# fenghansen/YOND_public

Measured on AMD Instinct MI355X. Metric: Bayer megapixels/sec end-to-end (NLE+VST+denoise+iVST), higher is better.
Workload: dtype f32 (3x3 convolutions: f32 operands as two f16 halves -- 22-23 significant bits -- on the f16 MFMA, 3 products per f32 product, f32 accumulate; per-layer error vs float64 asserted <= 2x the f32 direct kernel's and <= 2e-5 of max|ref| (tests/test_hip_conv.py; measured 1.3e-6 vs 1.5e-6), whole frame v

## Files before the change

yond_public_amd/csrc/conv_misc.hip:

```cpp
#include "common.h"

template <int TH>
__global__ __launch_bounds__(256) void conv_in_kernel(const float* __restrict__ x, const float* __restrict__ ub,
                                                      int H, int W, int Cout, const float* __restrict__ wpk,
                                                      const float* __restrict__ bias, float slope,
                                                      float* __restrict__ dst, int out_p4) {
    constexpr int IH = TH + 2, IW = 34, MW = TH / 4;
    __shared__ __attribute__((aligned(16))) float s_in[IH * IW * 4];
    __shared__ __attribute__((aligned(16))) float s_w[5 * 2 * 32 * 4];
    const int tid = threadIdx.x, lane = tid & 63, wave = tid >> 6, li = lane & 31, lh = lane >> 5;
    const int nct = Cout / 32;
    const int ntx = (W + 31) / 32;
    int b = blockIdx.x;
    const int ct = b % nct;
    b /= nct;
    const int tx = b % ntx, ty = b / ntx;
    const int n = blockIdx.y;
    const int ox0 = tx * 32, oy0 = ty * TH;
    const float u = ub ? ub[n] : 1.0f;
    for (int it = tid; it < IH * IW; it += 256) {
        const int py = it / IW, px = it % IW;
        const int gy = oy0 - 1 + py, gx = ox0 - 1 + px;
        f32x4 v = {0.0f, 0.0f, 0.0f, 0.0f};
        if (gy >= 0 && gy < H && gx >= 0 && gx < W) {
            v = *(const f32x4*)(x + ((size_t)(n * H + gy) * W + gx) * 4);
            if (ub) { v[0] /= u; v[1] /= u; v[2] /= u; v[3] /= u; }
        }
        *(f32x4*)(s_in + it * 4) = v;
    }
    for (int it = tid; it < 5 * 2 * 32; it += 256)
        *(f32x4*)(s_w + it * 4) = *(const f32x4*)(wpk + (size_t)ct * 1280 + it * 4);
    __syncthreads();

    f32x16 acc[MW];
#pragma unroll
    for (int m = 0; m < MW; ++m)
#pragma unroll
        for (int r = 0; r < 16; ++r) acc[m][r] = 0.0f;
#pragma unroll
    for (int up = 0; up < 5; ++up) {
        int tap = 2 * up + lh;
        if (tap > 8) tap = 8;
        const int dy = tap / 3, dx = tap % 3;
        const f32x4 bb = *(const f32x4*)(s_w + ((up * 2 + lh) * 32 + li) * 4);
#pragma unroll
        for (int m = 0; m < MW; ++m) {
            const f32x4 a = *(const f32x4*)(s_in + ((wave * MW + m + dy) * IW + li + dx) * 4);
#pragma unroll
            for (int t = 0; t < 4; ++t) acc[m] = __builtin_amdgcn_mfma_f32_32x32x2f32(bb[t], a[t], acc[m], 0, 0, 0);
        }
    }
    const int ox = ox0 + li;
#pragma unroll
    for (int m = 0; m < MW; ++m) {
        const int oy = oy0 + wave * MW + m;
        if (oy < H && ox < W) {
            float* op = out_p4 ? dst + (((size_t)n * (Cout / 4) + ct * 8 + lh) * H * W + (size_t)oy * W + ox) * 4
                               : dst + ((size_t)(n * H + oy) * W + ox) * Cout + ct * 32 + 4 * lh;
            const size_t gstep = out_p4 ? (size_t)8 * H * W : 8;
#pragma unroll
            for (int g = 0; g < 4; ++g) {
                const f32x4 zero = {0.0f, 0.0f, 0.0f, 0.0f};
                const f32x4 bv = bias ? *(const f32x4*)(bias + ct * 32 + 4 * lh + 8 * g) : zero;
                f32x4 v;
#pragma unroll
                for (int e = 0; e < 4; ++e) {
                    const float x = acc[m][4 * g + e] + bv[e];
                    v[e] = x > 0.0f ? x : x * slope;
                }
                *(f32x4*)(op + g * gstep) = v;
            }
        }
    }
}

extern "C" int yond_pack_conv_in_weight_f32(const float* w, int cout, float* dst) {
    if (!w || !dst || cout % 32 != 0) return YOND_EINVAL;
    size_t o = 0;
    for (int ct = 0; ct < cout / 32; ++ct)
        for (int up = 0; up < 5; ++up)
            for (int h = 0; h < 2; ++h)
                for (int j = 0; j < 32; ++j)
                    for (int e = 0; e < 4; ++e) {
                        const int tap = 2 * up + h, co = ct * 32 + j;
                        dst[o++] = tap < 9 ? w[((size_t)co * 4 + e) * 9 + tap] : 0.0f;
                    }
    return YOND_OK;
}

extern "C" int yond_conv_in_f32(const float* x, const float* ub, int N, int H, int W, int Cout, const float* wpk,
                                const float* bias, float slope, float* dst, int out_fmt, void* stream) {
    if (!x || !wpk || !dst || N <= 0 || H <= 0 || W <= 0 || N > 65535) return YOND_EINVAL;
    if (out_fmt != YOND_FMT_NHWC_F32 && out_fmt != YOND_FMT_PLANES4) return YOND_EINVAL;
    if (Cout % 32 != 0) return YOND_EUNSUPPORTED;
    constexpr int TH = 8;
    dim3 grid((Cout / 32) * ((W + 31) / 32) * ((H + TH - 1) / TH), N);
    hipLaunchKernelGGL(conv_in_kernel<TH>, grid, dim3(256), 0, (hipStream_t)stream, x, ub, H, W, Cout, wpk, bias, slope, dst,
                       out_fmt == YOND_FMT_PLANES4 ? 1 : 0);
    YOND_LAUNCH_CHECK();
    return YOND_OK;
}

__global__ __launch_bounds__(256) void conv_out_kernel(const float* __restrict__ feat, int Cin,
                                                       const float* __restrict__ w, const float* __restrict__ bias,
                                                       const float* __restrict__ x, const float* __restrict__ ub,
                                                       size_t npix_per_image, float* __restrict__ dst) {
    const int n = blockIdx.y;
    const int part = threadIdx.x & 7;
    const float u = ub ? ub[n] : 1.0f;
    const size_t stride = (size_t)gridDim.x * 32;
    for (size_t p = (size_t)blockIdx.x * 32 + (threadIdx.x >> 3); p < npix_per_image; p += stride) {
        const size_t gp = (size_t)n * npix_per_image + p;
        const float* f = feat + gp * Cin + part * 4;
        float o0 = 0.f, o1 = 0.f, o2 = 0.f, o3 = 0.f;
        for (int c = 0; c < Cin; c += 32) {
            const f32x4 v = *(const f32x4*)(f + c);
            const int cb = c + part * 4;
#pragma unroll
            for (int e = 0; e < 4; ++e) {
                o0 = fmaf(v[e], w[0 * Cin + cb + e], o0);
                o1 = fmaf(v[e], w[1 * Cin + cb + e], o1);
                o2 = fmaf(v[e], w[2 * Cin + cb + e], o2);
                o3 = fmaf(v[e], w[3 * Cin + cb + e], o3);
            }
        }
#pragma unroll
        for (int m = 1; m < 8; m <<= 1) {
            o0 += __shfl_xor(o0, m); o1 += __shfl_xor(o1, m); o2 += __shfl_xor(o2, m); o3 += __shfl_xor(o3, m);
        }
        if (part == 0) {
            if (bias) { o0 += bias[0]; o1 += bias[1]; o2 += bias[2]; o3 += bias[3]; }
            if (x) {
                f32x4 xv = *(const f32x4*)(x + gp * 4);
                if (ub) { xv[0] /= u; xv[1] /= u; xv[2] /= u; xv[3] /= u; }
                o0 += xv[0]; o1 += xv[1]; o2 += xv[2]; o3 += xv[3];
            }
            if (ub) { o0 *= u; o1 *= u; o2 *= u; o3 *= u; }
            f32x4 o = {o0, o1, o2, o3};
            *(f32x4*)(dst + gp * 4) = o;
        }
    }
}

extern "C" int yond_conv_out_f32(const float* feat, int Cin, const float* w, const float* bias, const float* x,
                                 const float* ub, int N, int H, int W, float* dst, void* stream) {
    if (!feat || !w || !dst || N <= 0 || H <= 0 || W <= 0 || N > 65535) return YOND_EINVAL;
    if (Cin % 32 != 0) return YOND_EUNSUPPORTED;
    const size_t npix = (size_t)H * W;
    size_t nb = (npix + 31) / 32;
    if (nb > 256 * 32) nb = 256 * 32;
    dim3 grid((unsigned)nb, N);
    hipLaunchKernelGGL(conv_out_kernel, grid, dim3(256), 0, (hipStream_t)stream, feat, Cin, w, bias, x, ub, npix, dst);
    YOND_LAUNCH_CHECK();
    return YOND_OK;
}

__global__ __launch_bounds__(256) void maxpool2_kernel(const float* __restrict__ src, int H, int W, int C,
                                                       float* __restrict__ dst, size_t total4) {
    const size_t i = (size_t)blockIdx.x * 256 + threadIdx.x;
    if (i >= total4) return;
    const int c4 = C / 4;
    const int Ho = H / 2, Wo = W / 2;
    const int c = (int)(i % c4);
    size_t p = i / c4;
    const int ox = (int)(p % Wo);
    p /= Wo;
    const int oy = (int)(p % Ho);
    const int n = (int)(p / Ho);
    const float* s = src + (((size_t)(n * H + 2 * oy) * W + 2 * ox) * C) + c * 4;
    const f32x4 a = *(const f32x4*)s, b2 = *(const f32x4*)(s + C);
    const f32x4 c2 = *(const f32x4*)(s + (size_t)W * C), d2 = *(const f32x4*)(s + (size_t)W * C + C);
    f32x4 o;
#pragma unroll
    for (int e = 0; e < 4; ++e) o[e] = fmaxf(fmaxf(a[e], b2[e]), fmaxf(c2[e], d2[e]));
    *(f32x4*)(dst + i * 4) = o;
}

extern "C" int yond_maxpool2_f32(const float* src, int N, int H, int W, int C, float* dst, void* stream) {
    if (!src || !dst || N <= 0 || H < 2 || W < 2 || (H & 1) || (W & 1) || C % 4 != 0) return YOND_EINVAL;
    const size_t total4 = (size_t)N * (H / 2) * (W / 2) * (C / 4);
    hipLaunchKernelGGL(maxpool2_kernel, dim3((unsigned)((total4 + 255) / 256)), dim3(256), 0, (hipStream_t)stream, src, H, W, C, dst, total4);
    YOND_LAUNCH_CHECK();
    return YOND_OK;
}

template <int STAGE>
__global__ __launch_bounds__(256) void film_kernel(const YondFilmDesc* __restrict__ descs, const float* __restrict__ t,
                                                   const float* __restrict__ ub) {
    __shared__ float s_h[1024];
    const YondFilmDesc d = descs[blockIdx.y];
    const int n = blockIdx.z;
    const int C = d.C;
    if ((int)blockIdx.x * 32 >= C) return;
    const int tid = threadIdx.x, lane = tid & 63, wave = tid >> 6;
    float tv = t[n];
    if (ub) tv = tv / ub[n];
    const float* Wm;
    if (STAGE == 0) {
        for (int c = tid; c < C; c += 256) s_h[c] = silu_f(fmaf(d.w_a0[c], tv, d.b_a0[c]));
        Wm = d.w_a2;
    } else {
        if (d.kind == 0) {
            for (int c = tid; c < C; c += 256) s_h[c] = silu_f(d.s1[(size_t)n * d.ld + c]);
        } else {
            for (int c = tid; c < C; c += 256) s_h[c] = silu_f(fmaf(d.w_b0[c], tv, d.b_b0[c]));
        }
        Wm = d.w_b;
    }
    __syncthreads();
    for (int row0 = blockIdx.x * 32; row0 < C; row0 += gridDim.x * 32) {
    float acc8[8];
#pragma unroll
    for (int i = 0; i < 8; ++i) acc8[i] = 0.0f;
    const int rbase = row0 + wave * 8;
    for (int j = lane; j < C; j += 64) {
        const float hj = s_h[j];
#pragma unroll
        for (int i = 0; i < 8; ++i) {
            const int row = min(rbase + i, C - 1);
            acc8[i] = fmaf(Wm[(size_t)row * C + j], hj, acc8[i]);
        }
    }
#pragma unroll
    for (int i = 0; i < 8; ++i) {
        const int row = rbase + i;
        float s = acc8[i];
#pragma unroll
        for (int o = 32; o > 0; o >>= 1) s += __shfl_xor(s, o);
        if (row >= C) continue;
        if (lane == 0) {
            const size_t o = (size_t)n * d.ld + row;
            if (STAGE == 0) {
                d.s1[o] = s + d.b_a2[row];
            } else {
                const float m2 = s + d.b_b[row];
                const float m1 = d.s1[o];
                if (d.kind == 0) {
                    d.t1[o] = fmaf(d.cb1[row], m1, m2);
                    d.s2[o] = 1.0f;
                    d.t2[o] = d.cb2[row];
                } else {
                    d.t1[o] = d.cb1[row] * m1;
                    d.s2[o] = m2;
                    d.t2[o] = d.cb2[row] * m2;
                }
            }
        }
    }
    }
}

extern "C" int yond_film_f32(const YondFilmDesc* descs, int nblocks, const float* t, const float* ub, int N, void* stream) {
    if (!descs || !t || nblocks <= 0 || N <= 0 || N > 65535 || nblocks > 65535) return YOND_EINVAL;
    dim3 grid(N >= 8 ? (unsigned)yond_exp_long("YOND_FILM_GX", 8) : 1024 / 32, nblocks, N);
    hipLaunchKernelGGL(film_kernel<0>, grid, dim3(256), 0, (hipStream_t)stream, descs, t, ub);
    YOND_LAUNCH_CHECK();
    hipLaunchKernelGGL(film_kernel<1>, grid, dim3(256), 0, (hipStream_t)stream, descs, t, ub);
    YOND_LAUNCH_CHECK();
    return YOND_OK;
}
```

Before: 2612.

## Make conv_in persistent with double-buffered input tiles and prefetch

```diff
diff --git a/yond_public_amd/csrc/conv_misc.hip b/yond_public_amd/csrc/conv_misc.hip
--- a/yond_public_amd/csrc/conv_misc.hip
+++ b/yond_public_amd/csrc/conv_misc.hip
@@ -1,76 +1,112 @@
 #include "common.h"
 
 template <int TH>
-__global__ __launch_bounds__(256) void conv_in_kernel(const float* __restrict__ x, const float* __restrict__ ub,
-                                                      int H, int W, int Cout, const float* __restrict__ wpk,
+__global__ __launch_bounds__(256) __attribute__((amdgpu_waves_per_eu(5, 5))) void conv_in_kernel(const float* __restrict__ x, const float* __restrict__ ub,
+                                                      int N, int H, int W, int Cout, const float* __restrict__ wpk,
                                                       const float* __restrict__ bias, float slope,
                                                       float* __restrict__ dst, int out_p4) {
     constexpr int IH = TH + 2, IW = 34, MW = TH / 4;
-    __shared__ __attribute__((aligned(16))) float s_in[IH * IW * 4];
-    __shared__ __attribute__((aligned(16))) float s_w[5 * 2 * 32 * 4];
+    constexpr int NLD = (IH * IW + 255) / 256;
+    __shared__ __attribute__((aligned(16))) float s_in[2][IH * IW * 4];
     const int tid = threadIdx.x, lane = tid & 63, wave = tid >> 6, li = lane & 31, lh = lane >> 5;
-    const int nct = Cout / 32;
-    const int ntx = (W + 31) / 32;
-    int b = blockIdx.x;
-    const int ct = b % nct;
-    b /= nct;
-    const int tx = b % ntx, ty = b / ntx;
-    const int n = blockIdx.y;
-    const int ox0 = tx * 32, oy0 = ty * TH;
-    const float u = ub ? ub[n] : 1.0f;
-    for (int it = tid; it < IH * IW; it += 256) {
-        const int py = it / IW, px = it % IW;
-        const int gy = oy0 - 1 + py, gx = ox0 - 1 + px;
-        f32x4 v = {0.0f, 0.0f, 0.0f, 0.0f};
-        if (gy >= 0 && gy < H && gx >= 0 && gx < W) {
-            v = *(const f32x4*)(x + ((size_t)(n * H + gy) * W + gx) * 4);
-            if (ub) { v[0] /= u; v[1] /= u; v[2] /= u; v[3] /= u; }
-        }
-        *(f32x4*)(s_in + it * 4) = v;
-    }
+    const int ct = blockIdx.y;
+    const int ntx = (W + 31) / 32, nty = (H + TH - 1) / TH;
+    const int per_img = ntx * nty, total = N * per_img;
+    int t = blockIdx.x;
+    if (t >= total) return;
+    __shared__ __attribute__((aligned(16))) float s_w[5 * 2 * 32 * 4 + 32];
     for (int it = tid; it < 5 * 2 * 32; it += 256)
         *(f32x4*)(s_w + it * 4) = *(const f32x4*)(wpk + (size_t)ct * 1280 + it * 4);
+    if (tid < 32) s_w[1280 + tid] = bias ? bias[ct * 32 + tid] : 0.0f;
+    struct Tile { int n, ox0, oy0; };
+    auto tile_of = [&](int tt) {
+        Tile r;
+        r.n = tt / per_img;
+        const int q = tt - r.n * per_img, ty = q / ntx;
+        r.ox0 = (q - ty * ntx) * 32;
+        r.oy0 = ty * TH;
+        return r;
+    };
+    f32x4 v[NLD];
+    float u = 1.0f;
+    auto fetch = [&](const Tile& tl) {
+#pragma unroll
+        for (int k = 0; k < NLD; ++k) {
+            const int it = min(tid + k * 256, IH * IW - 1);
+            const int py = it / IW, px = it % IW;
+            const int gy = min(max(tl.oy0 - 1 + py, 0), H - 1), gx = min(max(tl.ox0 - 1 + px, 0), W - 1);
+            v[k] = *(const f32x4*)(x + ((size_t)(tl.n * H + gy) * W + gx) * 4);
+        }
+        if (ub) u = ub[tl.n];
+    };
+    auto stage = [&](const Tile& tl, float* s) {
+#pragma unroll
+        for (int k = 0; k < NLD; ++k) {
+            const int it = tid + k * 256;
+            if (it >= IH * IW) continue;
+            const int py = it / IW, px = it % IW;
+            const int gy = tl.oy0 - 1 + py, gx = tl.ox0 - 1 + px;
+            f32x4 a = {0.0f, 0.0f, 0.0f, 0.0f};
+            if (gy >= 0 && gy < H && gx >= 0 && gx < W) {
+                a = v[k];
+                if (ub) { a[0] /= u; a[1] /= u; a[2] /= u; a[3] /= u; }
+            }
+            *(f32x4*)(s + it * 4) = a;
+        }
+    };
+    Tile cur = tile_of(t);
+    fetch(cur);
+    stage(cur, s_in[0]);
     __syncthreads();
-
-    f32x16 acc[MW];
-#pragma unroll
-    for (int m = 0; m < MW; ++m)
-#pragma unroll
-        for (int r = 0; r < 16; ++r) acc[m][r] = 0.0f;
-#pragma unroll
-    for (int up = 0; up < 5; ++up) {
-        int tap = 2 * up + lh;
-        if (tap > 8) tap = 8;
-        const int dy = tap / 3, dx = tap % 3;
-        const f32x4 bb = *(const f32x4*)(s_w + ((up * 2 + lh) * 32 + li) * 4);
+    for (int buf = 0;; buf ^= 1) {
+        const int tn = t + gridDim.x;
+        const Tile nxt = tile_of(tn);
+        if (tn < total) fetch(nxt);
+        const float* si = s_in[buf];
+        f32x16 acc[MW];
+#pragma unroll
+        for (int m = 0; m < MW; ++m)
+#pragma unroll
+            for (int r = 0; r < 16; ++r) acc[m][r] = 0.0f;
+#pragma unroll
+        for (int up = 0; up < 5; ++up) {
+            int tap = 2 * up + lh;
+            if (tap > 8) tap = 8;
+            const int dy = tap / 3, dx = tap % 3;
+            const f32x4 bb = *(const f32x4*)(s_w + ((up * 2 + lh) * 32 + li) * 4);
+#pragma unroll
+            for (int m = 0; m < MW; ++m) {
+                const f32x4 a = *(const f32x4*)(si + ((wave * MW + m + dy) * IW + li + dx) * 4);
+#pragma unroll
+                for (int e = 0; e < 4; ++e) acc[m] = __builtin_amdgcn_mfma_f32_32x32x2f32(bb[e], a[e], acc[m], 0, 0, 0);
+            }
+        }
+        if (tn < total) stage(nxt, s_in[buf ^ 1]);
+        const int ox = cur.ox0 + li;
 #pragma unroll
         for (int m = 0; m < MW; ++m) {
-            const f32x4 a = *(const f32x4*)(s_in + ((wave * MW + m + dy) * IW + li + dx) * 4);
-#pragma unroll
-            for (int t = 0; t < 4; ++t) acc[m] = __builtin_amdgcn_mfma_f32_32x32x2f32(bb[t], a[t], acc[m], 0, 0, 0);
-        }
-    }
-    const int ox = ox0 + li;
-#pragma unroll
-    for (int m = 0; m < MW; ++m) {
-        const int oy = oy0 + wave * MW + m;
-        if (oy < H && ox < W) {
-            float* op = out_p4 ? dst + (((size_t)n * (Cout / 4) + ct * 8 + lh) * H * W + (size_t)oy * W + ox) * 4
-                               : dst + ((size_t)(n * H + oy) * W + ox) * Cout + ct * 32 + 4 * lh;
-            const size_t gstep = out_p4 ? (size_t)8 * H * W : 8;
-#pragma unroll
-            for (int g = 0; g < 4; ++g) {
-                const f32x4 zero = {0.0f, 0.0f, 0.0f, 0.0f};
-                const f32x4 bv = bias ? *(const f32x4*)(bias + ct * 32 + 4 * lh + 8 * g) : zero;
-                f32x4 v;
-#pragma unroll
-                for (int e = 0; e < 4; ++e) {
-                    const float x = acc[m][4 * g + e] + bv[e];
-                    v[e] = x > 0.0f ? x : x * slope;
+            const int oy = cur.oy0 + wave * MW + m;
+            if (oy < H && ox < W) {
+                float* op = out_p4 ? dst + (((size_t)cur.n * (Cout / 4) + ct * 8 + lh) * H * W + (size_t)oy * W + ox) * 4
+                                   : dst + ((size_t)(cur.n * H + oy) * W + ox) * Cout + ct * 32 + 4 * lh;
+                const size_t gstep = out_p4 ? (size_t)8 * H * W : 8;
+#pragma unroll
+                for (int g = 0; g < 4; ++g) {
+                    const f32x4 bv = *(const f32x4*)(s_w + 1280 + 4 * lh + 8 * g);
+                    f32x4 o;
+#pragma unroll
+                    for (int e = 0; e < 4; ++e) {
+                        const float y = acc[m][4 * g + e] + bv[e];
+                        o[e] = y > 0.0f ? y : y * slope;
+                    }
+                    *(f32x4*)(op + g * gstep) = o;
                 }
-                *(f32x4*)(op + g * gstep) = v;
-            }
-        }
+            }
+        }
+        if (tn >= total) break;
+        __syncthreads();
+        t = tn;
+        cur = nxt;
     }
 }
 
@@ -94,8 +130,13 @@
     if (out_fmt != YOND_FMT_NHWC_F32 && out_fmt != YOND_FMT_PLANES4) return YOND_EINVAL;
     if (Cout % 32 != 0) return YOND_EUNSUPPORTED;
     constexpr int TH = 8;
-    dim3 grid((Cout / 32) * ((W + 31) / 32) * ((H + TH - 1) / TH), N);
-    hipLaunchKernelGGL(conv_in_kernel<TH>, grid, dim3(256), 0, (hipStream_t)stream, x, ub, H, W, Cout, wpk, bias, slope, dst,
+    const long long tiles = (long long)N * ((W + 31) / 32) * ((H + TH - 1) / TH);
+    if (tiles > (1LL << 30)) return YOND_EUNSUPPORTED;
+    long long slots = 256LL * yond_exp_long("YOND_CONV_IN_WGS", 5) / (Cout / 32);
+    if (slots < 1) slots = 1;
+    const long long per_wg = (tiles + slots - 1) / slots;
+    dim3 grid((unsigned)((tiles + per_wg - 1) / per_wg), Cout / 32);
+    hipLaunchKernelGGL(conv_in_kernel<TH>, grid, dim3(256), 0, (hipStream_t)stream, x, ub, N, H, W, Cout, wpk, bias, slope, dst,
                        out_fmt == YOND_FMT_PLANES4 ? 1 : 0);
     YOND_LAUNCH_CHECK();
     return YOND_OK;
```

New measurement: 2631, median of 6. Within noise of the previous version (+0.7%).
